# jluuser/PyTorch-VAE

Hardware: AMD Instinct MI355X
Metric: train images/sec @64x64x3 bs256 (curve tensors [B,64,6], SURVEY.md s0) (higher is better)
Workload: dtype f32; 1 GPU; C2: stage2_vq.yaml model with num_quantizers=1 K=512 D=64 N=64; full train step (fwd+loss+bwd+clip+AdamW+EMA), dropout 0.1, loss weights at epoch 100; per_gpu_batch=256, global_batch=256, seq_len=64, parallelism=dp1, hipgraph=True, params=43115078

## Files before the change

### pytorch-vae_amd/csrc/gemm.hip

```cpp
#include "common.h"
#include <type_traits>
#include <utility>
#include <vector>
#include <algorithm>

namespace {

constexpr int BM = 128, BN = 128;
constexpr int BK = 32;
template <int BKT> struct Tile {
    static constexpr int KC_LD = BKT + 4;
    static constexpr int A_TILE = BM * KC_LD;
    static constexpr int NLD = BKT / 8;
};

enum EpiMode {
    EPI_LINEAR = 0,
    EPI_RELU_DROP = 1,
    EPI_GELU = 2,
    EPI_DROP_RESID = 3,
    EPI_SIGMOID = 4,
    EPI_MUL_POSMASK = 5,
    EPI_MUL_GELUGRAD = 6,
    EPI_MUL_SIGGRAD = 7,
// ... 578 lines not shown
                        const float am = A[(size_t)(r + u * slices) * lda + m];
                        acc[m] += am * bv[u];
                        asum[m] += am;
                    }
        }
        for (; r < r1; r += slices) {
            const f32x4 bv = *reinterpret_cast<const f32x4*>(B + (size_t)r * ldb + q * 4);
#pragma unroll
            for (int m = 0; m < M; ++m) {
                    const float am = A[(size_t)r * lda + m];
                    acc[m] += am * bv;
                    asum[m] += am;
                }
        }
#pragma unroll
        for (int m = 0; m < M; ++m) {
                *reinterpret_cast<f32x4*>(red + ((size_t)sl * M + m) * N + q * 4) = acc[m];
                if (q == 0) red_rs[sl][m] = asum[m];
            }
    }
    __syncthreads();
    float* out = slab + (size_t)blockIdx.x * M * N;
    for (int i = threadIdx.x; i < M * nq; i += 256) {
        f32x4 v = *reinterpret_cast<const f32x4*>(red + (size_t)i * 4);
        for (int s2 = 1; s2 < slices; ++s2) v += *reinterpret_cast<const f32x4*>(red + (size_t)s2 * M * N + (size_t)i * 4);
        *reinterpret_cast<f32x4*>(out + (size_t)i * 4) = v;
    }
    if (rs && threadIdx.x < M) {
        float t = 0.f;
        for (int s2 = 0; s2 < slices; ++s2) t += red_rs[s2][threadIdx.x];
        rs[(size_t)blockIdx.x * M + threadIdx.x] = t;
    }
}

#include "gemm_dma.inc"
#include "gemm_p3.inc"

struct ProfRec { int slot; double flops; hipEvent_t e0, e1; };
bool g_prof_on = false;
std::vector<ProfRec> g_prof;
constexpr int PROF_MODES = 9;
constexpr int PROF_FAMILIES = 7;
inline int prof_slot(bool a_kc, bool b_kc, int mode_t, int family = 0) {
    return (family * 4 + (a_kc ? 2 : 0) + (b_kc ? 1 : 0)) * PROF_MODES + mode_t + 1;
}

template <bool A_KC, bool B_KC, int BKT, int MODE = -1>
int launch(const GemmArgs& g, int splits, hipStream_t stream) {
    static bool attr_set = false;
    const size_t smem = (size_t)4 * Tile<BKT>::A_TILE * sizeof(float);
    if (!attr_set) {
        hipError_t e = hipFuncSetAttribute(reinterpret_cast<const void*>(&gemm_f32_mfma<A_KC, B_KC, BKT, MODE>),
                                           hipFuncAttributeMaxDynamicSharedMemorySize, (int)smem);
        if (e != hipSuccess) {
            vqh_set_error(hipGetErrorString(e));
            return VQH_ERR_LAUNCH;
        }
        attr_set = true;
    }
    const int tiles = ((g.M + BM - 1) / BM) * ((g.N + BN - 1) / BN);
    dim3 grid(tiles, 1, splits);
    ProfRec rec{};
    if (g_prof_on) {
        rec.slot = prof_slot(A_KC, B_KC, MODE);
        rec.flops = 2.0 * g.M * g.N * g.K;
        if (hipEventCreate(&rec.e0) != hipSuccess || hipEventCreate(&rec.e1) != hipSuccess ||
            hipEventRecord(rec.e0, stream) != hipSuccess) {
            vqh_set_error("vqh_gemm: profiling events failed");
            return VQH_ERR_LAUNCH;
        }
    }
    hipLaunchKernelGGL((gemm_f32_mfma<A_KC, B_KC, BKT, MODE>), grid, dim3(256), smem, stream, g);
    VQH_LAUNCH_CHECK();
    if (g_prof_on) {
        if (hipEventRecord(rec.e1, stream) != hipSuccess) {
            vqh_set_error("vqh_gemm: profiling events failed");
            return VQH_ERR_LAUNCH;
        }
        g_prof.push_back(rec);
    }
    return VQH_OK;
}

template <bool A_KC, bool B_KC, int MODE, bool X3>
int launch_dma_impl(const GemmArgs& g, int splits, hipStream_t stream) {
    static bool attr_set = false;
    auto kern = X3 ? &gemm_f32_x3<A_KC, B_KC, MODE> : &gemm_f32_dma<A_KC, B_KC, MODE>;
    if (!attr_set) {
        hipError_t e = hipFuncSetAttribute(reinterpret_cast<const void*>(kern),
                                           hipFuncAttributeMaxDynamicSharedMemorySize, dma::LDS_BYTES);
        if (e != hipSuccess) {
            vqh_set_error(hipGetErrorString(e));
            return VQH_ERR_LAUNCH;
        }
        attr_set = true;
    }
    dim3 grid((g.M / dma::TBM) * (g.N / dma::TBN), 1, splits);
    ProfRec rec{};
    if (g_prof_on) {
        rec.slot = prof_slot(A_KC, B_KC, MODE, X3 ? 3 : 1);
        rec.flops = 2.0 * g.M * g.N * g.K;
        if (hipEventCreate(&rec.e0) != hipSuccess || hipEventCreate(&rec.e1) != hipSuccess ||
            hipEventRecord(rec.e0, stream) != hipSuccess) {
            vqh_set_error("vqh_gemm: profiling events failed");
            return VQH_ERR_LAUNCH;
        }
    }
    hipLaunchKernelGGL(kern, grid, dim3(256), dma::LDS_BYTES, stream, g);
    VQH_LAUNCH_CHECK();
    if (g_prof_on) {
        if (hipEventRecord(rec.e1, stream) != hipSuccess) {
            vqh_set_error("vqh_gemm: profiling events failed");
            return VQH_ERR_LAUNCH;
        }
        g_prof.push_back(rec);
    }
    return VQH_OK;
}

template <bool A_KC, bool B_KC, int MODE = -1>
int launch_dma(const GemmArgs& g, int splits, hipStream_t stream) {
    if (g.flags & 512) return launch_dma_impl<A_KC, B_KC, MODE, false>(g, splits, stream);
    return launch_dma_impl<A_KC, B_KC, MODE, true>(g, splits, stream);
}

}

extern "C" int vqh_gemm_profile_begin(void) {
    g_prof.clear();
    g_prof_on = true;
    return VQH_OK;
}
extern "C" int vqh_gemm_profile_end(double* out) {
    g_prof_on = false;
    if (out)
        for (int i = 0; i < PROF_FAMILIES * 4 * PROF_MODES * 3; ++i) out[i] = 0.0;
    int rc = VQH_OK;
    for (ProfRec& r : g_prof) {
        float ms = 0.f;
        if (hipEventSynchronize(r.e1) != hipSuccess || hipEventElapsedTime(&ms, r.e0, r.e1) != hipSuccess) {
            vqh_set_error("vqh_gemm_profile_end: event query failed");
            rc = VQH_ERR_LAUNCH;
        } else if (out) {
            out[r.slot * 3 + 0] += 1.0;
            out[r.slot * 3 + 1] += (double)ms * 1e-3;
            out[r.slot * 3 + 2] += r.flops;
        }
        (void)hipEventDestroy(r.e0);
        (void)hipEventDestroy(r.e1);
    }
    g_prof.clear();
    return rc;
}

extern "C" int vqh_reduce_slabs(const float* slabs, int S, long long stride, long long n, float* out, float beta,
                                hipStream_t stream);

static int g_gemm_flags = 1;
extern "C" int vqh_gemm_set_flags(int flags) {
#ifndef VQH_DIAG
    flags &= ~(2 | 4);
#endif
    const int old = g_gemm_flags; g_gemm_flags = flags; return old;
}

static int gemm_impl(int a_kcontig, int b_kcontig, int M, int N, int K, const float* A, int lda, const float* B,
                     int ldb, float* C, int ldc, const float* bias, int mode, const float* aux_in, float* aux_out,
                     int ldaux, float beta, const unsigned long long* rng_state, unsigned drop_site, float drop_p,
                     float* workspace, long long workspace_floats, float* rowsum, hipStream_t stream) {
    VQH_CHECK_ARG(M >= 0 && N >= 0 && K >= 0, "vqh_gemm: negative dimension");
    if (M == 0 || N == 0) return VQH_OK;
    VQH_CHECK_ARG(C && ((A && B) || K == 0), "vqh_gemm: null operand");
    VQH_CHECK_ARG(mode >= EPI_LINEAR && mode <= EPI_MUL_SIGGRAD, "vqh_gemm: unknown epilogue mode");
    VQH_CHECK_ARG(lda >= (a_kcontig ? K : M) && ldb >= (b_kcontig ? K : N) && ldc >= N, "vqh_gemm: leading dim too small");
    if (mode == EPI_GELU) VQH_CHECK_ARG(aux_out && ldaux >= N, "vqh_gemm: GELU epilogue needs aux_out");
    if (mode == EPI_DROP_RESID || mode >= EPI_MUL_POSMASK)
        VQH_CHECK_ARG(aux_in && ldaux >= N, "vqh_gemm: epilogue needs aux_in");
    VQH_CHECK_ARG(drop_p >= 0.f && drop_p < 1.f, "vqh_gemm: dropout p out of range");
    if (drop_p > 0.f && (mode == EPI_RELU_DROP || mode == EPI_DROP_RESID))
        VQH_CHECK_ARG(rng_state != nullptr, "vqh_gemm: dropout needs rng_state");

    GemmArgs g;
    g.A = A; g.B = B; g.C = C;
    g.M = M; g.N = N; g.K = K;
    g.lda = lda; g.ldb = ldb; g.ldc = ldc;
    g.vecA = ((reinterpret_cast<uintptr_t>(A) & 15) == 0 && (lda & 3) == 0) ? 1 : 0;
    g.vecB = ((reinterpret_cast<uintptr_t>(B) & 15) == 0 && (ldb & 3) == 0) ? 1 : 0;
    {
        uintptr_t al = reinterpret_cast<uintptr_t>(C) | reinterpret_cast<uintptr_t>(bias) | reinterpret_cast<uintptr_t>(aux_in) |
                       reinterpret_cast<uintptr_t>(aux_out);
        g.vecC = ((al & 15) == 0 && (ldc & 3) == 0 && ((aux_in || aux_out) ? (ldaux & 3) == 0 : true) && (N & 3) == 0) ? 1 : 0;
    }
    g.mode = mode; g.bias = bias; g.aux_in = aux_in; g.aux_out = aux_out; g.ldaux = ldaux; g.beta = beta;
    g.drop = make_drop(rng_state, drop_site, drop_p);
    g.ws = nullptr;
    g.rowsum = rowsum;
    g.rowsum_ws = nullptr;
    g.flags = g_gemm_flags;
    if (rowsum) VQH_CHECK_ARG(!a_kcontig && mode == EPI_LINEAR, "vqh_gemm_wgrad: row sums need the [K,M] A layout and a linear epilogue");

    if (!(g_gemm_flags & 64)) {
        auto al16 = [](const void* p_) { return (reinterpret_cast<uintptr_t>(p_) & 15) == 0; };
        if (mode == EPI_LINEAR && !rowsum && a_kcontig && b_kcontig && N <= SK_MAX && K >= 64 && (K & 3) == 0 &&
            (lda & 3) == 0 && (ldb & 3) == 0 && al16(A) && al16(B)) {
            int blocks = (M + 3) / 4;
            if (blocks > 2048) blocks = 2048;
#define SK_CASE(V) case V: hipLaunchKernelGGL(skinny_n_kernel<V>, dim3(blocks), dim3(256), 0, stream, A, lda, B, ldb, C, ldc, bias, beta, M, K); break
            switch (N) { SK_CASE(1); SK_CASE(2); SK_CASE(3); SK_CASE(4); SK_CASE(5); SK_CASE(6); SK_CASE(7); default: SK_CASE(8); }
#undef SK_CASE
            VQH_LAUNCH_CHECK();
            return VQH_OK;
        }
        if (mode == EPI_LINEAR && !rowsum && !bias && a_kcontig && !b_kcontig && K <= SK_MAX && K > 0 && N >= 64 &&
            (N & 3) == 0 && (ldb & 3) == 0 && (ldc & 3) == 0 && al16(B) && al16(C)) {
            const long long quads = (long long)M * (N >> 2);
            int blocks = (int)((quads + 255) / 256);
            if (blocks > 4096) blocks = 4096;
#define SK_CASE(V) case V: hipLaunchKernelGGL(skinny_k_kernel<V>, dim3(blocks), dim3(256), 0, stream, A, lda, B, ldb, C, ldc, beta, M, N); break
            switch (K) { SK_CASE(1); SK_CASE(2); SK_CASE(3); SK_CASE(4); SK_CASE(5); SK_CASE(6); SK_CASE(7); default: SK_CASE(8); }
#undef SK_CASE
            VQH_LAUNCH_CHECK();
            return VQH_OK;
        }
        if (mode == EPI_LINEAR && !a_kcontig && !b_kcontig && M <= SK_MAX && N >= 64 && (N & 3) == 0 && (ldb & 3) == 0 &&
            (ldc & 3) == 0 && al16(B) && al16(C) && al16(workspace) && !bias && workspace && K >= 256 && N <= 1024 &&
            256 % (N >> 2) == 0) {
            const int rows_per_block = 64;
            const int nblk = (K + rows_per_block - 1) / rows_per_block;
            const long long per = (long long)M * N + (rowsum ? M : 0);
            if ((long long)nblk * per <= workspace_floats && ldc == N) {
                float* rs_ws = rowsum ? workspace + (size_t)nblk * M * N : nullptr;
#define SK_CASE(V) case V: hipLaunchKernelGGL(skinny_m_kernel<V>, dim3(nblk), dim3(256), 0, stream, A, lda, B, ldb, workspace, rs_ws, N, K, rows_per_block); break
                switch (M) { SK_CASE(1); SK_CASE(2); SK_CASE(3); SK_CASE(4); SK_CASE(5); SK_CASE(6); SK_CASE(7); default: SK_CASE(8); }
#undef SK_CASE
                VQH_LAUNCH_CHECK();
                int rc2 = vqh_reduce_slabs(workspace, nblk, (long long)M * N, (long long)M * N, C, beta, stream);
                if (rc2 == VQH_OK && rowsum) rc2 = vqh_reduce_slabs(rs_ws, nblk, (long long)M, (long long)M, rowsum, beta, stream);
                return rc2;
            }
        }
    }

    if (!(g_gemm_flags & 128) && (M % dma::TBM) == 0 && (N % dma::TBN) == 0 && (K % dma::TBK) == 0 && K >= dma::TBK && g.vecA &&
        g.vecB && g.vecC && (!rowsum || (reinterpret_cast<uintptr_t>(workspace) & 15) == 0)) {
        const int tiles_d = (M / dma::TBM) * (N / dma::TBN);
        int splits_d = 1;
        if (workspace && mode == EPI_LINEAR && tiles_d < 192 && K >= 8 * dma::TBK) {
            splits_d = 256 / tiles_d;
            const int max_by_k = K / (4 * dma::TBK);
            if (splits_d > max_by_k) splits_d = max_by_k;
            const long long per = (long long)M * N + (rowsum ? M : 0);
            if ((long long)splits_d * per > workspace_floats) splits_d = (int)(workspace_floats / per);
            if (splits_d < 2) splits_d = 1;
        }
        int kchunk_d = ((K + splits_d - 1) / splits_d + dma::TBK - 1) / dma::TBK * dma::TBK;
        splits_d = (K + kchunk_d - 1) / kchunk_d;
        const bool pairs_fit = (long long)M * N / 2 < (1LL << 32);
        if (tiles_d * splits_d >= 96 && pairs_fit) {
            g.kchunk = kchunk_d;
            if (splits_d > 1) {
                g.ws = workspace;
                if (rowsum) g.rowsum_ws = workspace + (size_t)splits_d * M * N;
            }
            int rc;
            if (a_kcontig && b_kcontig) {
                if (splits_d == 1 && mode == EPI_DROP_RESID) rc = launch_dma<true, true, EPI_DROP_RESID>(g, splits_d, stream);
                else if (splits_d == 1 && mode == EPI_RELU_DROP) rc = launch_dma<true, true, EPI_RELU_DROP>(g, splits_d, stream);
                else if (splits_d == 1 && mode == EPI_GELU) rc = launch_dma<true, true, EPI_GELU>(g, splits_d, stream);
                else if (mode == EPI_LINEAR) rc = launch_dma<true, true, EPI_LINEAR>(g, splits_d, stream);
                else rc = launch_dma<true, true>(g, splits_d, stream);
            } else if (a_kcontig && !b_kcontig) {
                if (splits_d == 1 && mode == EPI_MUL_POSMASK) rc = launch_dma<true, false, EPI_MUL_POSMASK>(g, splits_d, stream);
                else if (splits_d == 1 && mode == EPI_MUL_GELUGRAD) rc = launch_dma<true, false, EPI_MUL_GELUGRAD>(g, splits_d, stream);
                else if (mode == EPI_LINEAR) rc = launch_dma<true, false, EPI_LINEAR>(g, splits_d, stream);
                else rc = launch_dma<true, false>(g, splits_d, stream);
            } else if (!a_kcontig && b_kcontig) {
                if (mode == EPI_LINEAR) rc = launch_dma<false, true, EPI_LINEAR>(g, splits_d, stream);
                else rc = launch_dma<false, true>(g, splits_d, stream);
            } else {
                if (mode == EPI_LINEAR) rc = launch_dma<false, false, EPI_LINEAR>(g, splits_d, stream);
                else rc = launch_dma<false, false>(g, splits_d, stream);
            }
            if (rc != VQH_OK) return rc;
            if (splits_d > 1) {
                const size_t total = (size_t)M * N;
                int blocks = (int)((total / 4 + 255) / 256);
                if (blocks > 4096) blocks = 4096;
                if (rowsum && blocks < (M + 255) / 256) blocks = (M + 255) / 256;
                hipLaunchKernelGGL(splitk_reduce_vec, dim3(blocks), dim3(256), 0, stream, workspace, splits_d, M, N, C, ldc, bias,
                                   beta, g.rowsum_ws, rowsum);
                VQH_LAUNCH_CHECK();
            }
            return VQH_OK;
        }
        g.ws = nullptr;
        g.rowsum_ws = nullptr;
    }

    const int tiles = ((M + BM - 1) / BM) * ((N + BN - 1) / BN);
    int splits = 1;
    if (workspace && mode == EPI_LINEAR && tiles < 256 && K >= 8 * BK) {
        splits = 512 / tiles;
        const int max_by_k = K / (4 * BK);
        if (splits > max_by_k) splits = max_by_k;
        const long long per = (long long)M * N + (rowsum ? M : 0);
        if ((long long)splits * per > workspace_floats) splits = (int)(workspace_floats / per);
        if (splits < 2) splits = 1;
    }
    int kchunk = ((K + splits - 1) / splits + BK - 1) / BK * BK;
    if (kchunk <= 0) kchunk = BK;
    splits = (K + kchunk - 1) / kchunk;
    if (splits < 1) splits = 1;
    g.kchunk = kchunk;
    if (splits > 1) {
        g.ws = workspace;
        if (rowsum) g.rowsum_ws = workspace + (size_t)splits * M * N;
    }

    int rc;
    if (splits == 1 && g.vecC && a_kcontig && b_kcontig && mode == EPI_DROP_RESID) {
        rc = launch<true, true, 32, EPI_DROP_RESID>(g, splits, stream);
    } else if (splits == 1 && g.vecC && a_kcontig && b_kcontig && mode == EPI_RELU_DROP) {
        rc = launch<true, true, 32, EPI_RELU_DROP>(g, splits, stream);
    } else if (splits == 1 && g.vecC && a_kcontig && b_kcontig && mode == EPI_GELU) {
        rc = launch<true, true, 32, EPI_GELU>(g, splits, stream);
    } else if (splits == 1 && g.vecC && a_kcontig && !b_kcontig && mode == EPI_MUL_POSMASK) {
        rc = launch<true, false, 32, EPI_MUL_POSMASK>(g, splits, stream);
    } else if (splits == 1 && g.vecC && a_kcontig && !b_kcontig && mode == EPI_MUL_GELUGRAD) {
        rc = launch<true, false, 32, EPI_MUL_GELUGRAD>(g, splits, stream);
    } else {
        if (a_kcontig && b_kcontig) rc = launch<true, true, 32>(g, splits, stream);
        else if (a_kcontig && !b_kcontig) rc = launch<true, false, 32>(g, splits, stream);
        else if (!a_kcontig && b_kcontig) rc = launch<false, true, 32>(g, splits, stream);
        else rc = launch<false, false, 32>(g, splits, stream);
    }
    if (rc != VQH_OK) return rc;
    if (splits > 1) {
        const size_t total = (size_t)M * N;
        int blocks = (int)((total + 255) / 256);
        if (blocks > 2048) blocks = 2048;
        if (rowsum && blocks < (M + 255) / 256) blocks = (M + 255) / 256;
// ... 522 lines not shown
```

### pytorch-vae_amd/csrc/gemm_dma.inc

```

namespace dma {
constexpr int TBM = 256, TBN = 128, TBK = 32;
constexpr int A_BYTES = TBM * TBK * 4, B_BYTES = TBN * TBK * 4, STAGE_BYTES = A_BYTES + B_BYTES;
constexpr int NSTAGE = 3, LDS_BYTES = NSTAGE * STAGE_BYTES;
constexpr int DMA_A = A_BYTES / 1024 / 4, DMA_B = B_BYTES / 1024 / 4, DMA_PER_WAVE = DMA_A + DMA_B;
constexpr int MI = 4, NJ = 2;
}

typedef float f32x2 __attribute__((ext_vector_type(2)));

typedef unsigned u32x2 __attribute__((ext_vector_type(2)));
typedef unsigned u32x4 __attribute__((ext_vector_type(4)));
typedef short s16x4 __attribute__((ext_vector_type(4)));
typedef __bf16 bf16x8 __attribute__((ext_vector_type(8)));

namespace x3 {
constexpr int A_PLANE = dma::TBM * dma::TBK * 2, B_PLANE = dma::TBN * dma::TBK * 2;
constexpr int B_OFF = 3 * A_PLANE;
constexpr int STAGE_BYTES = 3 * (A_PLANE + B_PLANE);
constexpr int LDS_BYTES = 2 * STAGE_BYTES;
constexpr int NU = 12, NUA = 8;
constexpr int NB = 8, G = 48, NSLOT = 96;
constexpr int BAR = 7 * NU;
constexpr int RS_OFF = 40960;
static_assert(LDS_BYTES <= dma::LDS_BYTES, "x3 stages must fit the launch's dynamic LDS");
}

template <class F, int... I>
__device__ __forceinline__ void static_for_impl(F&& f, std::integer_sequence<int, I...>) { (f(std::integral_constant<int, I>{}), ...); }
template <int N, class F>
__device__ __forceinline__ void static_for(F&& f) { static_for_impl(f, std::make_integer_sequence<int, N>{}); }

struct SplitUnit {
    float r0, r1, r2, r3;
    unsigned t0, t1, t2, t3;
    unsigned hp[2], mp[2], lp[2];
    template <int S> __device__ __forceinline__ void step(const f32x4& a) {
        if constexpr (S == 0) {
            asm volatile("v_cvt_pk_bf16_f32 %0, %6, %7\n\tv_cvt_pk_bf16_f32 %1, %8, %9\n\tv_lshlrev_b32 %2, 16, %0\n\t"
                         "v_and_b32 %3, 0xffff0000, %0\n\tv_sub_f32 %4, %6, %2\n\tv_sub_f32 %5, %7, %3"
                         : "=&v"(hp[0]), "=&v"(hp[1]), "=&v"(t0), "=&v"(t1), "=&v"(r0), "=&v"(r1)
                         : "v"(a[0]), "v"(a[1]), "v"(a[2]), "v"(a[3]) : "memory");
        } else if constexpr (S == 1) {
            asm volatile("v_lshlrev_b32 %0, 16, %6\n\tv_and_b32 %1, 0xffff0000, %6\n\tv_sub_f32 %2, %7, %0\n\t"
                         "v_sub_f32 %3, %8, %1\n\tv_cvt_pk_bf16_f32 %4, %9, %10\n\tv_cvt_pk_bf16_f32 %5, %2, %3"
                         : "=&v"(t2), "=&v"(t3), "=&v"(r2), "=&v"(r3), "=&v"(mp[0]), "=&v"(mp[1])
                         : "v"(hp[1]), "v"(a[2]), "v"(a[3]), "v"(r0), "v"(r1) : "memory");
        } else if constexpr (S == 2) {
            asm volatile("v_lshlrev_b32 %0, 16, %2\n\tv_and_b32 %1, 0xffff0000, %2" : "=&v"(t0), "=&v"(t1) : "v"(mp[0]) : "memory");
        } else if constexpr (S == 3) {
            asm volatile("v_sub_f32 %0, %0, %2\n\tv_sub_f32 %1, %1, %3" : "+v"(r0), "+v"(r1) : "v"(t0), "v"(t1) : "memory");
        } else if constexpr (S == 4) {
            asm volatile("v_lshlrev_b32 %0, 16, %6\n\tv_and_b32 %1, 0xffff0000, %6\n\tv_sub_f32 %2, %2, %0\n\t"
                         "v_sub_f32 %3, %3, %1\n\tv_cvt_pk_bf16_f32 %4, %7, %8\n\tv_cvt_pk_bf16_f32 %5, %2, %3"
                         : "=&v"(t2), "=&v"(t3), "+v"(r2), "+v"(r3), "=&v"(lp[0]), "=&v"(lp[1])
                         : "v"(mp[1]), "v"(r0), "v"(r1) : "memory");
        }
    }
    __device__ __forceinline__ void all(const f32x4& a) { step<0>(a); step<1>(a); step<2>(a); step<3>(a); step<4>(a); }
};

__device__ __forceinline__ void glds16_s(const char* ubase, unsigned voff, unsigned lds_byte_addr_uniform) {
    asm volatile("s_mov_b32 m0, %2\n\ts_nop 0\n\tglobal_load_lds_dwordx4 %0, %1"
                 :
                 : "v"(voff), "s"(ubase), "s"(lds_byte_addr_uniform)
                 : "memory");
}

__device__ __forceinline__ void glds16(const float* gptr, unsigned lds_byte_addr_uniform) {
    __builtin_amdgcn_global_load_lds(gptr, (__attribute__((address_space(3))) void*)(uintptr_t)lds_byte_addr_uniform, 16, 0, 0);
}

template <bool A_KC, bool B_KC, int MODE, bool X3 = false>
__device__ __forceinline__ void gemm_dma_tile(const GemmArgs& g, const int tile, const int zsplit) {
    using namespace dma;
    constexpr bool EA_KC = X3 ? true : A_KC, EB_KC = X3 ? true : B_KC;
    extern __shared__ __attribute__((aligned(1024))) unsigned char smem_dma[];
    const int tid = threadIdx.x, lane = tid & 63;
    const int wave = __builtin_amdgcn_readfirstlane(tid >> 6);
    const int wm = wave >> 1, wn = wave & 1;
    const int l31 = lane & 31, h = lane >> 5;

    const int tiles_n = g.N / TBN;
    const int m0 = (tile / tiles_n) * TBM, n0 = (tile % tiles_n) * TBN;
    const int kbeg = zsplit * g.kchunk;
    const int kend = min(g.K, kbeg + g.kchunk);
    const int nk = (kend - kbeg) / TBK;

    unsigned voff[DMA_PER_WAVE];
    unsigned dst[DMA_PER_WAVE];
#pragma unroll
    for (int i = 0; i < DMA_A; ++i) {
        const int j = wave + 4 * i;
        if (A_KC) {
            const int R = j * 8 + (lane >> 3), c = (lane & 7) ^ ((R >> 1) & 7);
            voff[i] = (unsigned)(((size_t)R * g.lda + c * 4) * 4);
        } else {
            voff[i] = (unsigned)(((size_t)j * g.lda + lane * 4) * 4);
        }
        dst[i] = j * 1024;
    }
#pragma unroll
    for (int i = 0; i < DMA_B; ++i) {
        const int j = wave + 4 * i;
        if (B_KC) {
            const int R = j * 8 + (lane >> 3), c = (lane & 7) ^ ((R >> 1) & 7);
            voff[DMA_A + i] = (unsigned)(((size_t)R * g.ldb + c * 4) * 4);
        } else {
            voff[DMA_A + i] = (unsigned)(((size_t)(2 * j + (lane >> 5)) * g.ldb + (lane & 31) * 4) * 4);
        }
        dst[DMA_A + i] = A_BYTES + j * 1024;
    }
    const char* baseA = reinterpret_cast<const char*>(A_KC ? g.A + (size_t)m0 * g.lda + kbeg : g.A + (size_t)kbeg * g.lda + m0);
    const char* baseB = reinterpret_cast<const char*>(B_KC ? g.B + (size_t)n0 * g.ldb + kbeg : g.B + (size_t)kbeg * g.ldb + n0);
    const size_t stepA = (A_KC ? (size_t)TBK : (size_t)TBK * g.lda) * 4;
    const size_t stepB = (B_KC ? (size_t)TBK : (size_t)TBK * g.ldb) * 4;
    const unsigned lds0 = (unsigned)(uintptr_t)smem_dma;

    const int sw = (l31 >> 1) & 7;
    unsigned offA[4], offB[4];
#pragma unroll
    for (int t = 0; t < 4; ++t) {
        offA[t] = A_KC ? (unsigned)((wm * 128 + l31) * 128 + (((2 * t + h) ^ sw) * 16))
                       : (unsigned)((8 * t + 4 * h) * (TBM * 4) + (wm * 128 + 4 * l31) * 4);
        offB[t] = A_BYTES + (B_KC ? (unsigned)((wn * 64 + l31) * 128 + (((2 * t + h) ^ sw) * 16))
                                  : (unsigned)((8 * t + 4 * h) * (TBN * 4) + (wn * 64 + 2 * l31) * 4));
    }

    f32x16 acc[MI][NJ];
#pragma unroll
    for (int i = 0; i < MI; ++i)
#pragma unroll
        for (int j = 0; j < NJ; ++j)
#pragma unroll
            for (int r = 0; r < 16; ++r) acc[i][j][r] = 0.f;

    f32x4 fa[2][4];
    f32x4 fbk[2][2];
    f32x2 fbr[2][4];
    const bool do_rowsum = (!A_KC) && (g.rowsum != nullptr) && (n0 == 0) && (X3 || wn == 0);
    float rs[4] = {0.f, 0.f, 0.f, 0.f};

    constexpr int NREAD = 4 + (B_KC ? 2 : 4);
    constexpr int NMF = 4 * MI * NJ;
    constexpr int GAP = NMF / (NREAD + 1);
    auto substep = [&](auto c_c, auto rt_c, auto v0_c, auto v1_c, int rstage, int kt_d, int dstage) {
        constexpr int c = decltype(c_c)::value, RT = decltype(rt_c)::value, V0 = decltype(v0_c)::value,
                      V1 = decltype(v1_c)::value, n = c ^ 1;
        const unsigned char* sb = smem_dma + rstage * STAGE_BYTES;
        const unsigned dsb = lds0 + dstage * STAGE_BYTES;
        if (do_rowsum) {
#pragma unroll
            for (int e = 0; e < 4; ++e)
#pragma unroll
                for (int i = 0; i < 4; ++i) rs[i] += fa[c][e][i];
        }
#pragma unroll
        for (int m = 0; m < NMF; ++m) {
            const int e = m / (MI * NJ), i = (m / NJ) % MI, j = m % NJ;
            const float av = A_KC ? fa[c][i][e] : fa[c][e][i];
            const float bv = B_KC ? fbk[c][j][e] : fbr[c][e][j];
            acc[i][j] = __builtin_amdgcn_mfma_f32_32x32x2f32(av, bv, acc[i][j], 0, 0, 0);
            if ((m % GAP) == 0 && m / GAP < NREAD) {
                const int d = m / GAP;
                if (d < 4) {
                    fa[n][d] = *reinterpret_cast<const f32x4*>(sb + offA[RT] + (A_KC ? d * 32 * 128 : d * TBM * 4));
                } else if (B_KC) {
                    fbk[n][d - 4] = *reinterpret_cast<const f32x4*>(sb + offB[RT] + (d - 4) * 32 * 128);
                } else {
                    fbr[n][d - 4] = *reinterpret_cast<const f32x2*>(sb + offB[RT] + (d - 4) * TBN * 4);
                }
            }
            if ((m % GAP) == GAP / 2 && V0 + m / GAP < V1) {
                const int v = V0 + m / GAP;
                const char* ub = (v < DMA_A) ? baseA + (size_t)kt_d * stepA : baseB + (size_t)kt_d * stepB;
                glds16_s(ub, voff[v], __builtin_amdgcn_readfirstlane(dsb + dst[v]));
            }
        }
#pragma unroll
        for (int m = 0; m < NMF; ++m) {
            __builtin_amdgcn_sched_group_barrier(0x008, 1, 0);
            if ((m % GAP) == 0 && m / GAP < NREAD) __builtin_amdgcn_sched_group_barrier(0x100, 1, 0);
            if ((m % GAP) == GAP / 2 && V0 + m / GAP < V1) __builtin_amdgcn_sched_group_barrier(0x020, 1, 0);
        }
    };
    auto read_first = [&](int rstage) {
        const unsigned char* sb = smem_dma + rstage * STAGE_BYTES;
#pragma unroll
        for (int d = 0; d < 4; ++d) fa[0][d] = *reinterpret_cast<const f32x4*>(sb + offA[0] + (A_KC ? d * 32 * 128 : d * TBM * 4));
        if (B_KC) {
#pragma unroll
            for (int d = 0; d < 2; ++d) fbk[0][d] = *reinterpret_cast<const f32x4*>(sb + offB[0] + d * 32 * 128);
        } else {
#pragma unroll
            for (int d = 0; d < 4; ++d) fbr[0][d] = *reinterpret_cast<const f32x2*>(sb + offB[0] + d * TBN * 4);
        }
    };
    auto issue_all = [&](int kt, int stage) {
        const unsigned sbb = lds0 + stage * STAGE_BYTES;
#pragma unroll
        for (int v = 0; v < DMA_PER_WAVE; ++v) {
            const char* ub = (v < DMA_A) ? baseA + (size_t)kt * stepA : baseB + (size_t)kt * stepB;
            glds16_s(ub, voff[v], __builtin_amdgcn_readfirstlane(sbb + dst[v]));
        }
    };

    const int c4 = (lane & 15) * 4;
    const int col = n0 + wn * 64 + c4;
    constexpr bool HAS_DROP = (MODE == EPI_RELU_DROP || MODE == EPI_DROP_RESID);
    constexpr bool HAS_AUX = (MODE == EPI_DROP_RESID || MODE > EPI_SIGMOID);
    unsigned dkey = 0;
    if (g.drop.p > 0.f && g.drop.rng_state) dkey = drop_key(g.drop, g.drop.rng_state[0], g.drop.rng_state[1]);
    unsigned dmask[4] = {0u, 0u, 0u, 0u};
    const unsigned pair0 = (unsigned)((((unsigned long long)(m0 + wm * 128 + (lane >> 4)) * g.N + col) >> 2) * 2);
    const unsigned g0 = pair0 * 0x9E3779B9U;
    const unsigned gstep = (unsigned)(2 * g.N) * 0x9E3779B9U;
    auto hash_quad = [&](int qi) {
        const unsigned gq = g0 + (unsigned)qi * gstep;
        const unsigned b0 = mix32(dkey ^ gq), b1 = mix32(dkey ^ (gq + 0x9E3779B9U));
        unsigned f4 = ((b0 & 0xffffu) >= g.drop.thr) ? 1u : 0u;
        f4 |= ((b0 >> 16) >= g.drop.thr) ? 2u : 0u;
        f4 |= ((b1 & 0xffffu) >= g.drop.thr) ? 4u : 0u;
        f4 |= ((b1 >> 16) >= g.drop.thr) ? 8u : 0u;
        const unsigned sh = f4 << ((qi & 7) * 4);
        const int w = qi >> 3;
#pragma unroll
        for (int k = 0; k < 4; ++k) dmask[k] |= (w == k) ? sh : 0u;
    };
    f32x4 auxr[32];
    auto load_aux_all = [&]() {
        const float* ap = g.aux_in + (size_t)(m0 + wm * 128 + (lane >> 4)) * g.ldaux + col;
#pragma unroll
        for (int q = 0; q < 32; ++q) auxr[q] = *reinterpret_cast<const f32x4*>(ap + (size_t)(q * 4) * g.ldaux);
    };

    using I0 = std::integral_constant<int, 0>;
    using I1 = std::integral_constant<int, 1>;
    using I2 = std::integral_constant<int, 2>;
    using I3 = std::integral_constant<int, 3>;
    using IH = std::integral_constant<int, DMA_PER_WAVE / 2>;
    using IF = std::integral_constant<int, DMA_PER_WAVE>;
    if constexpr (X3) {
        const unsigned vA = A_KC ? (unsigned)(((size_t)(8 * wave + (lane >> 3)) * g.lda + 4 * (lane & 7)) * 4)
                                 : (unsigned)(((size_t)(8 * wave) * g.lda + 4 * lane) * 4);
        const unsigned vB = B_KC ? (unsigned)(((size_t)(8 * wave + (lane >> 3)) * g.ldb + 4 * (lane & 7)) * 4)
                                 : (unsigned)(((size_t)(8 * wave + (lane >> 5)) * g.ldb + 4 * (lane & 31)) * 4);
        const size_t uA = (A_KC ? (size_t)32 * g.lda : (size_t)g.lda) * 4;
        const size_t uB = (B_KC ? (size_t)32 * g.ldb : (size_t)2 * g.ldb) * 4;
        unsigned wA[4], wB[2];
        {
            const int R = 8 * wave + (lane >> 3), c = (lane & 7) >> 1;
            const unsigned wkc = (unsigned)(R * 64 + ((c ^ ((R >> 2) & 3)) * 16) + (lane & 1) * 8);
#pragma unroll
            for (int x = 0; x < 4; ++x) wA[x] = A_KC ? wkc : (unsigned)((8 * wave) * 512 + (((lane >> 3) ^ x) * 64) + (lane & 7) * 8);
#pragma unroll
            for (int x = 0; x < 2; ++x)
                wB[x] = B_KC ? wkc
                             : (unsigned)((8 * wave + (lane >> 5)) * 256 + ((((lane >> 3) & 3) ^ ((2 * x + (lane >> 5)) & 3)) * 64) + (lane & 7) * 8);
        }
        unsigned rA[4], rB[2];
        {
            const int q = (lane & 15) >> 2, p = lane & 3, sub = (lane >> 4) & 1;
            if (A_KC) {
                const int R = wm * 128 + l31, f = (l31 >> 2) & 3;
                rA[0] = (unsigned)(R * 64 + ((h ^ f) * 16));
                rA[1] = (unsigned)(R * 64 + (((2 + h) ^ f) * 16));
                rA[2] = rA[3] = 0;
            } else {
#pragma unroll
                for (int i = 0; i < 4; ++i) rA[i] = (unsigned)((8 * h + q) * 512 + (((wm * 4 + i) ^ q) * 64) + (16 * sub + 4 * p) * 2);
            }
            if (B_KC) {
                const int R = wn * 64 + l31, f = (l31 >> 2) & 3;
                rB[0] = (unsigned)(R * 64 + ((h ^ f) * 16));
                rB[1] = (unsigned)(R * 64 + (((2 + h) ^ f) * 16));
            } else {
#pragma unroll
                for (int j = 0; j < 2; ++j) rB[j] = (unsigned)((8 * h + q) * 256 + (((wn * 2 + j) ^ q) * 64) + (16 * sub + 4 * p) * 2);
            }
        }
        f32x4 st[x3::NU];
        u32x4 xA[3][4];
        u32x4 xB[2][3][2];
        SplitUnit su;
        auto load_unit = [&](auto u_c, int kt) {
            constexpr int u = decltype(u_c)::value;
            if constexpr (u < x3::NUA) st[u] = *reinterpret_cast<const f32x4*>(baseA + (size_t)kt * stepA + (size_t)u * uA + vA);
            else st[u] = *reinterpret_cast<const f32x4*>(baseB + (size_t)kt * stepB + (size_t)(u - x3::NUA) * uB + vB);
        };
        auto write_unit = [&](auto u_c, auto pl_c, unsigned char* sb) {
            constexpr int u = decltype(u_c)::value, pl = decltype(pl_c)::value;
            const u32x2 v = pl == 0 ? u32x2{su.hp[0], su.hp[1]} : pl == 1 ? u32x2{su.mp[0], su.mp[1]} : u32x2{su.lp[0], su.lp[1]};
            if constexpr (u < x3::NUA) {
                constexpr int cst = A_KC ? u * 2048 : u * 512;
                *reinterpret_cast<u32x2*>(sb + pl * x3::A_PLANE + cst + wA[A_KC ? 0 : (u & 3)]) = v;
            } else {
                constexpr int i = u - x3::NUA;
                constexpr int cst = B_KC ? i * 2048 : 2 * i * 256;
                *reinterpret_cast<u32x2*>(sb + x3::B_OFF + pl * x3::B_PLANE + cst + wB[B_KC ? 0 : (i & 1)]) = v;
            }
        };
        auto read_A = [&](auto pl_c, auto i_c, auto g_c, const unsigned char* sb) -> u32x4 {
            constexpr int pl = decltype(pl_c)::value, i = decltype(i_c)::value, gg = decltype(g_c)::value;
            if constexpr (A_KC) {
                return *reinterpret_cast<const u32x4*>(sb + pl * x3::A_PLANE + i * 2048 + rA[gg]);
            } else {
                const unsigned a0 = (unsigned)(uintptr_t)(sb + pl * x3::A_PLANE + (16 * gg) * 512 + rA[i]);
                const s16x4 lo = __builtin_amdgcn_ds_read_tr16_b64_v4i16((__attribute__((address_space(3))) s16x4*)(uintptr_t)a0);
                const s16x4 hi = __builtin_amdgcn_ds_read_tr16_b64_v4i16((__attribute__((address_space(3))) s16x4*)(uintptr_t)(a0 + 4 * 512));
                const u32x2 l2 = __builtin_bit_cast(u32x2, lo), h2 = __builtin_bit_cast(u32x2, hi);
                return u32x4{l2[0], l2[1], h2[0], h2[1]};
            }
        };
        auto read_B = [&](auto pl_c, auto j_c, auto g_c, const unsigned char* sb) -> u32x4 {
            constexpr int pl = decltype(pl_c)::value, j = decltype(j_c)::value, gg = decltype(g_c)::value;
            if constexpr (B_KC) {
                return *reinterpret_cast<const u32x4*>(sb + x3::B_OFF + pl * x3::B_PLANE + j * 2048 + rB[gg]);
            } else {
                const unsigned a0 = (unsigned)(uintptr_t)(sb + x3::B_OFF + pl * x3::B_PLANE + (16 * gg) * 256 + rB[j]);
                const s16x4 lo = __builtin_amdgcn_ds_read_tr16_b64_v4i16((__attribute__((address_space(3))) s16x4*)(uintptr_t)a0);
                const s16x4 hi = __builtin_amdgcn_ds_read_tr16_b64_v4i16((__attribute__((address_space(3))) s16x4*)(uintptr_t)(a0 + 4 * 256));
                const u32x2 l2 = __builtin_bit_cast(u32x2, lo), h2 = __builtin_bit_cast(u32x2, hi);
                return u32x4{l2[0], l2[1], h2[0], h2[1]};
            }
        };
        auto aux_one = [&](auto q_c) {
            constexpr int q = decltype(q_c)::value;
            auxr[q] = *reinterpret_cast<const f32x4*>(g.aux_in + (size_t)(m0 + wm * 128 + (lane >> 4) + q * 4) * g.ldaux + col);
        };
        if (nk > 0) {
            static_for<x3::NU>([&](auto u_c) { load_unit(u_c, 0); });
            if (HAS_DROP && g.drop.p > 0.f && !g.ws) {
#pragma unroll
                for (int qi = 0; qi < 32; ++qi) hash_quad(qi);
            }
            static_for<x3::NU>([&](auto u_c) {
                constexpr int u = decltype(u_c)::value;
                if (do_rowsum && u < x3::NUA) {
#pragma unroll
                    for (int e = 0; e < 4; ++e) rs[e] += st[u][e];
                }
                su.all(st[u]);
                write_unit(u_c, I0{}, smem_dma);
                write_unit(u_c, I1{}, smem_dma);
                write_unit(u_c, I2{}, smem_dma);
                load_unit(u_c, nk > 1 ? 1 : 0);
            });
            asm volatile("s_waitcnt lgkmcnt(0)" ::: "memory");
            __builtin_amdgcn_s_barrier();
            static_for<4>([&](auto i_c) { xA[0][decltype(i_c)::value] = read_A(I0{}, i_c, I0{}, smem_dma); });
            static_for<6>([&](auto x_c) {
                constexpr int x = decltype(x_c)::value;
                xB[0][x / 2][x % 2] = read_B(std::integral_constant<int, x / 2>{}, std::integral_constant<int, x % 2>{}, I0{}, smem_dma);
            });
            auto kstep = [&](auto last_c, const int kt) {
                constexpr bool LAST = decltype(last_c)::value;
                const unsigned char* rstg = smem_dma + (kt & 1) * x3::STAGE_BYTES;
                unsigned char* wstg = smem_dma + ((kt & 1) ^ 1) * x3::STAGE_BYTES;
                const int kt_ld = min(kt + 2, nk - 1);
                const bool want_aux = LAST && HAS_AUX && !g.ws;
                static_for<x3::NSLOT>([&](auto m_c) {
                    constexpr int m = decltype(m_c)::value;
                    constexpr int gg = m / x3::G, mm = m % x3::G, pi = mm / x3::NB, b = mm % x3::NB, i = b / 2, j = b % 2;
                    constexpr int pa = (pi < 3) ? 0 : (pi < 5) ? 1 : 2;
                    constexpr int pb = (pi == 0 || pi == 3 || pi == 5) ? 0 : (pi == 1 || pi == 4) ? 1 : 2;
                    acc[i][j] = __builtin_amdgcn_mfma_f32_32x32x16_bf16(__builtin_bit_cast(bf16x8, xA[pa][i]),
                                                                        __builtin_bit_cast(bf16x8, xB[gg][pb][j]), acc[i][j], 0, 0, 0);
                    if constexpr (m < 8 && m % 2 == 0) xA[1][m / 2] = read_A(I1{}, std::integral_constant<int, m / 2>{}, I0{}, rstg);
                    if constexpr (m >= 8 && m < 16 && m % 2 == 0) xA[2][(m - 8) / 2] = read_A(I2{}, std::integral_constant<int, (m - 8) / 2>{}, I0{}, rstg);
                    if constexpr (m >= 16 && m < 28 && m % 2 == 0) {
                        constexpr int x = (m - 16) / 2;
                        xB[1][x / 2][x % 2] = read_B(std::integral_constant<int, x / 2>{}, std::integral_constant<int, x % 2>{}, I1{}, rstg);
                    }
                    if constexpr (m >= 28 && m < 44 && m % 4 == 0) xA[0][(m - 28) / 4] = read_A(I0{}, std::integral_constant<int, (m - 28) / 4>{}, I1{}, rstg);
                    if constexpr (m >= 48 && m < 56 && m % 2 == 0) xA[1][(m - 48) / 2] = read_A(I1{}, std::integral_constant<int, (m - 48) / 2>{}, I1{}, rstg);
                    if constexpr (m >= 56 && m < 64 && m % 2 == 0) xA[2][(m - 56) / 2] = read_A(I2{}, std::integral_constant<int, (m - 56) / 2>{}, I1{}, rstg);
                    if constexpr (!LAST) {
                        if constexpr (m >= x3::BAR && m < x3::BAR + 4) xA[0][m - x3::BAR] = read_A(I0{}, std::integral_constant<int, m - x3::BAR>{}, I0{}, wstg);
                        if constexpr (m >= x3::BAR + 4 && m < x3::BAR + 10) {
                            constexpr int x = m - x3::BAR - 4;
                            xB[0][x / 2][x % 2] = read_B(std::integral_constant<int, x / 2>{}, std::integral_constant<int, x % 2>{}, I0{}, wstg);
                        }
                        if constexpr (m < x3::BAR) {
                            constexpr int u = m / 7, ph = m % 7;
                            using U = std::integral_constant<int, u>;
                            if constexpr (ph == 0) {
                                if (do_rowsum && u < x3::NUA) {
#pragma unroll
                                    for (int e = 0; e < 4; ++e) rs[e] += st[u][e];
                                }
                                su.template step<0>(st[u]);
                            }
                            if constexpr (ph == 1) su.template step<1>(st[u]);
                            if constexpr (ph == 2) { su.template step<2>(st[u]); write_unit(U{}, I0{}, wstg); }
                            if constexpr (ph == 3) { su.template step<3>(st[u]); write_unit(U{}, I1{}, wstg); }
                            if constexpr (ph == 4) load_unit(U{}, kt_ld);
                            if constexpr (ph == 5) su.template step<4>(st[u]);
                            if constexpr (ph == 6) write_unit(U{}, I2{}, wstg);
                        }
                        if constexpr (m == x3::BAR - 1) {
                            asm volatile("s_waitcnt lgkmcnt(0)" ::: "memory");
                            __builtin_amdgcn_s_barrier();
                        }
                    } else if constexpr (HAS_AUX) {
                        if constexpr (m % 3 == 0) {
                            if (want_aux) aux_one(std::integral_constant<int, m / 3>{});
                        }
                    }
                    __builtin_amdgcn_sched_barrier(0);
                });
            };
            for (int kt = 0; kt < nk - 1; ++kt) kstep(std::false_type{}, kt);
            kstep(std::true_type{}, nk - 1);
            __builtin_amdgcn_s_barrier();
        } else if (HAS_AUX && !g.ws) {
            load_aux_all();
        }
    } else
    if (nk > 0) {
        issue_all(0, 0);
        issue_all(nk > 1 ? 1 : 0, 1);
        if (HAS_DROP && g.drop.p > 0.f && !g.ws) {
#pragma unroll
            for (int qi = 0; qi < 32; ++qi) hash_quad(qi);
        }
        asm volatile("s_waitcnt vmcnt(%0)" ::"n"(DMA_PER_WAVE) : "memory");
        __builtin_amdgcn_s_barrier();
        read_first(0);
        int stage = 0;
        for (int kt = 0; kt < nk; ++kt) {
            const int nxt = (stage == 2) ? 0 : stage + 1;
            const int nx2 = (nxt == 2) ? 0 : nxt + 1;
            if (HAS_AUX && !g.ws && kt == nk - 1) load_aux_all();
            substep(I0{}, I1{}, I0{}, I0{}, stage, 0, 0);
            substep(I1{}, I2{}, I0{}, I0{}, stage, 0, 0);
            asm volatile("s_waitcnt vmcnt(0)" ::: "memory");
            __builtin_amdgcn_s_barrier();
            const int ktd = min(kt + 2, nk - 1);
            substep(I0{}, I3{}, I0{}, IH{}, stage, ktd, nx2);
            substep(I1{}, I0{}, IH{}, IF{}, nxt, ktd, nx2);
            stage = nxt;
        }
        asm volatile("s_waitcnt vmcnt(0)" ::: "memory");
        __builtin_amdgcn_s_barrier();
    } else if (HAS_AUX && !g.ws) {
        load_aux_all();
    }

    if (X3 && do_rowsum) {
        float* rsb = reinterpret_cast<float*>(smem_dma + x3::RS_OFF);
        *reinterpret_cast<f32x4*>(rsb + wave * TBM + 4 * lane) = f32x4{rs[0], rs[1], rs[2], rs[3]};
        __builtin_amdgcn_s_barrier();
        if (wave == 0) {
            f32x4 t = *reinterpret_cast<const f32x4*>(rsb + 4 * lane);
#pragma unroll
            for (int w = 1; w < 4; ++w) t += *reinterpret_cast<const f32x4*>(rsb + w * TBM + 4 * lane);
            const int row = m0 + 4 * lane;
            if (g.rowsum_ws) {
                *reinterpret_cast<f32x4*>(g.rowsum_ws + (size_t)zsplit * g.M + row) = t;
            } else {
#pragma unroll
                for (int i = 0; i < 4; ++i) g.rowsum[row + i] = (g.beta != 0.f) ? g.beta * g.rowsum[row + i] + t[i] : t[i];
            }
        }
    } else
    if (do_rowsum) {
#pragma unroll
        for (int i = 0; i < 4; ++i) rs[i] += __shfl_xor(rs[i], 32, 64);
        if (h == 0) {
            const int row = m0 + wm * 128 + 4 * l31;
            if (g.rowsum_ws) {
                *reinterpret_cast<f32x4*>(g.rowsum_ws + (size_t)zsplit * g.M + row) = f32x4{rs[0], rs[1], rs[2], rs[3]};
            } else {
#pragma unroll
                for (int i = 0; i < 4; ++i)
                    g.rowsum[row + i] = (g.beta != 0.f) ? g.beta * g.rowsum[row + i] + rs[i] : rs[i];
            }
        }
    }

    const int mode = (MODE >= 0) ? MODE : g.mode;
    constexpr int EP_LD = 68;
    float* ep = reinterpret_cast<float*>(smem_dma) + wave * (32 * EP_LD);
    float* slab = g.ws ? g.ws + (size_t)zsplit * g.M * g.N : nullptr;
    if constexpr (X3 && MODE == EPI_LINEAR) {
        if (!(g.flags & 2048)) {
            const size_t ldo = slab ? (size_t)g.N : (size_t)g.ldc;
            float* obase = slab ? slab : g.C;
#pragma unroll
            for (int j = 0; j < NJ; ++j) {
                const int cj = n0 + wn * 64 + j * 32 + l31;
                const float bj = (g.bias && !slab) ? g.bias[cj] : 0.f;
                float* cp = obase + (size_t)(m0 + wm * 128 + 4 * h) * ldo + cj;
                if (!slab && g.beta != 0.f) {
#pragma unroll
                    for (int i = 0; i < MI; ++i)
#pragma unroll
                        for (int r = 0; r < 16; ++r) {
                            float* q = cp + (size_t)(i * 32 + (r & 3) + 8 * (r >> 2)) * ldo;
                            *q = acc[i][j][r] + bj + g.beta * *q;
                        }
                } else {
#pragma unroll
                    for (int i = 0; i < MI; ++i)
#pragma unroll
                        for (int r = 0; r < 16; ++r) cp[(size_t)(i * 32 + (r & 3) + 8 * (r >> 2)) * ldo] = acc[i][j][r] + bj;
                }
            }
            return;
        }
    }
    f32x4 bias4 = {0.f, 0.f, 0.f, 0.f};
    if (mode <= EPI_SIGMOID && g.bias && !slab) bias4 = *reinterpret_cast<const f32x4*>(g.bias + col);
#pragma unroll
    for (int grp = 0; grp < 4; ++grp) {
        __builtin_amdgcn_wave_barrier();
#pragma unroll
        for (int q = 0; q < 16; ++q) {
            int rr, i, r;
            if (EA_KC) { i = grp; r = q; rr = (q & 3) + 8 * (q >> 2) + 4 * h; }
            else { i = q >> 2; r = 4 * grp + (q & 3); rr = 4 * ((q & 3) + 4 * h) + i; }
            if (EB_KC) {
                ep[rr * EP_LD + l31] = acc[i][0][r];
                ep[rr * EP_LD + 32 + l31] = acc[i][1][r];
            } else {
                *reinterpret_cast<f32x2*>(ep + rr * EP_LD + 2 * l31) = f32x2{acc[i][0][r], acc[i][1][r]};
            }
        }
        __builtin_amdgcn_s_waitcnt(0xC07F);
        __builtin_amdgcn_wave_barrier();
        constexpr int EPI_UNROLL = (MODE >= 0) ? 8 : 1;
#pragma unroll EPI_UNROLL
        for (int it = 0; it < 8; ++it) {
            const int rl = it * 4 + (lane >> 4);
            const int row = m0 + wm * 128 + grp * 32 + rl;
            f32x4 v = *reinterpret_cast<const f32x4*>(ep + rl * EP_LD + c4);
            if (slab) {
                *reinterpret_cast<f32x4*>(slab + (size_t)row * g.N + col) = v;
                continue;
            }
            float* cptr = g.C + (size_t)row * g.ldc + col;
            if (mode <= EPI_SIGMOID) {
                v += bias4;
                if (mode == EPI_RELU_DROP || mode == EPI_DROP_RESID) {
                    if (mode == EPI_RELU_DROP)
#pragma unroll
                        for (int e = 0; e < 4; ++e) v[e] = fmaxf(v[e], 0.f);
                    if (g.drop.p > 0.f) {
                        if (HAS_DROP) {
#pragma unroll
                            for (int e = 0; e < 4; ++e) v[e] = ((dmask[grp] >> (it * 4 + e)) & 1u) ? v[e] * g.drop.scale : 0.f;
                        } else {
                            float f[4];
                            drop4(g.drop, dkey, ((unsigned long long)row * g.N + col) >> 2, f);
#pragma unroll
                            for (int e = 0; e < 4; ++e) v[e] *= f[e];
                        }
                    }
                    if (mode == EPI_DROP_RESID)
                        v += HAS_AUX ? auxr[grp * 8 + it] : *reinterpret_cast<const f32x4*>(g.aux_in + (size_t)row * g.ldaux + col);
                } else if (mode == EPI_GELU) {
                    *reinterpret_cast<f32x4*>(g.aux_out + (size_t)row * g.ldaux + col) = v;
#pragma unroll
                    for (int e = 0; e < 4; ++e) v[e] = gelu_erf(v[e]);
                } else if (mode == EPI_SIGMOID) {
#pragma unroll
                    for (int e = 0; e < 4; ++e) v[e] = 1.f / (1.f + __expf(-v[e]));
                }
            } else {
                const f32x4 a = HAS_AUX ? auxr[grp * 8 + it] : *reinterpret_cast<const f32x4*>(g.aux_in + (size_t)row * g.ldaux + col);
                if (mode == EPI_MUL_POSMASK) {
#pragma unroll
                    for (int e = 0; e < 4; ++e) v[e] = (a[e] > 0.f) ? v[e] * g.drop.scale : 0.f;
                } else if (mode == EPI_MUL_GELUGRAD) {
#pragma unroll
                    for (int e = 0; e < 4; ++e) v[e] *= gelu_erf_grad(a[e]);
                } else {
#pragma unroll
                    for (int e = 0; e < 4; ++e) v[e] *= a[e] * (1.f - a[e]);
                }
            }
            if (g.beta != 0.f) v += g.beta * *reinterpret_cast<const f32x4*>(cptr);
            *reinterpret_cast<f32x4*>(cptr) = v;
        }
        __builtin_amdgcn_s_waitcnt(0xC07F);
    }
}

template <bool A_KC, bool B_KC, int MODE>
__global__ __launch_bounds__(256, 1) void gemm_f32_dma(const GemmArgs g) {
    const int nx = gridDim.x, nt = nx * gridDim.z, lin = blockIdx.z * nx + blockIdx.x;
    const int q = nt >> 3, r = nt & 7, x = lin & 7, j = lin >> 3;
    const int v = (x < r ? x * (q + 1) : r * (q + 1) + (x - r) * q) + j;
    gemm_dma_tile<A_KC, B_KC, MODE>(g, v % nx, v / nx);
}

template <bool A_KC, bool B_KC, int MODE>
__global__ __launch_bounds__(256, 1) void gemm_f32_x3(const GemmArgs g) {
    const int nx = gridDim.x, nt = nx * gridDim.z, lin = blockIdx.z * nx + blockIdx.x;
    const int q = nt >> 3, r = nt & 7, x = lin & 7, j = lin >> 3;
    const int v = (x < r ? x * (q + 1) : r * (q + 1) + (x - r) * q) + j;
    gemm_dma_tile<A_KC, B_KC, MODE, true>(g, v % nx, v / nx);
}

constexpr int GROUP_MAX = 8;
struct GemmGroupArgs {
    int n;
    int wg_begin[GROUP_MAX + 1];
    int tiles[GROUP_MAX];
    GemmArgs p[GROUP_MAX];
};

__device__ __forceinline__ int group_logical_id() {
    const int nt = gridDim.x, lin = blockIdx.x;
    const int q = nt >> 3, r = nt & 7, x = lin & 7, j = lin >> 3;
    return (x < r ? x * (q + 1) : r * (q + 1) + (x - r) * q) + j;
}

__global__ __launch_bounds__(256, 1) void gemm_f32_dma_group(const GemmGroupArgs G) {
    const int v = ((G.p[0].flags & 1) && !(G.p[0].flags & 1024)) ? group_logical_id() : (int)blockIdx.x;
    int p = 0;
    while (p + 1 < G.n && v >= G.wg_begin[p + 1]) ++p;
    const int local = v - G.wg_begin[p];
    const int tiles = G.tiles[p];
    gemm_dma_tile<false, false, EPI_LINEAR>(G.p[p], local % tiles, local / tiles);
}
__global__ __launch_bounds__(256, 1) void gemm_f32_x3_group(const GemmGroupArgs G) {
    const int v = ((G.p[0].flags & 1) && !(G.p[0].flags & 1024)) ? group_logical_id() : (int)blockIdx.x;
    int p = 0;
    while (p + 1 < G.n && v >= G.wg_begin[p + 1]) ++p;
    const int local = v - G.wg_begin[p];
    const int tiles = G.tiles[p];
    gemm_dma_tile<false, false, EPI_LINEAR, true>(G.p[p], local % tiles, local / tiles);
}
```

Measured before the change: 9289 images/s.

## Add register-direct epilogue for x3 GEMM ReLU-dropout and GELU modes

For the x3 (bf16x3 split) DMA GEMM path with RELU_DROP or GELU epilogues, results are now written straight from accumulator registers to global memory instead of being staged through LDS. The dropout hash is computed per unit and interleaved into the last k-step's MFMA schedule, with masks exchanged between lane pairs via DPP. The final barrier is skipped. The old LDS-staged path stays available as a separate kernel behind a flag. A second flag can force the DMA path for small tile counts. This trades the LDS round trip and barrier for uncoalesced strided global stores, plus extra registers and hash work inside the main loop.

```diff
diff --git a/pytorch-vae_amd/csrc/gemm.hip b/pytorch-vae_amd/csrc/gemm.hip
--- a/pytorch-vae_amd/csrc/gemm.hip
+++ b/pytorch-vae_amd/csrc/gemm.hip
@@ -684,10 +684,13 @@
     return VQH_OK;
 }
 
-template <bool A_KC, bool B_KC, int MODE, bool X3>
+template <bool A_KC, bool B_KC, int MODE, bool X3, bool STAGED = false>
 int launch_dma_impl(const GemmArgs& g, int splits, hipStream_t stream) {
     static bool attr_set = false;
-    auto kern = X3 ? &gemm_f32_x3<A_KC, B_KC, MODE> : &gemm_f32_dma<A_KC, B_KC, MODE>;
+    void (*kern)(const GemmArgs);
+    if constexpr (!X3) kern = &gemm_f32_dma<A_KC, B_KC, MODE>;
+    else if constexpr (STAGED) kern = &gemm_f32_x3_staged<A_KC, B_KC, MODE>;
+    else kern = &gemm_f32_x3<A_KC, B_KC, MODE>;
     if (!attr_set) {
         hipError_t e = hipFuncSetAttribute(reinterpret_cast<const void*>(kern),
                                            hipFuncAttributeMaxDynamicSharedMemorySize, dma::LDS_BYTES);
@@ -723,6 +726,9 @@
 template <bool A_KC, bool B_KC, int MODE = -1>
 int launch_dma(const GemmArgs& g, int splits, hipStream_t stream) {
     if (g.flags & 512) return launch_dma_impl<A_KC, B_KC, MODE, false>(g, splits, stream);
+    if constexpr (x3_register_epilogue(MODE)) {
+        if (g.flags & 2048) return launch_dma_impl<A_KC, B_KC, MODE, true, true>(g, splits, stream);
+    }
     return launch_dma_impl<A_KC, B_KC, MODE, true>(g, splits, stream);
 }
 
@@ -858,7 +864,7 @@
         int kchunk_d = ((K + splits_d - 1) / splits_d + dma::TBK - 1) / dma::TBK * dma::TBK;
         splits_d = (K + kchunk_d - 1) / kchunk_d;
         const bool pairs_fit = (long long)M * N / 2 < (1LL << 32);
-        if (tiles_d * splits_d >= 96 && pairs_fit) {
+        if ((tiles_d * splits_d >= 96 || (g_gemm_flags & 4096)) && pairs_fit) {
             g.kchunk = kchunk_d;
             if (splits_d > 1) {
                 g.ws = workspace;
diff --git a/pytorch-vae_amd/csrc/gemm_dma.inc b/pytorch-vae_amd/csrc/gemm_dma.inc
--- a/pytorch-vae_amd/csrc/gemm_dma.inc
+++ b/pytorch-vae_amd/csrc/gemm_dma.inc
@@ -8,6 +8,7 @@
 }
 
 typedef float f32x2 __attribute__((ext_vector_type(2)));
+constexpr bool x3_register_epilogue(int mode) { return mode == EPI_RELU_DROP || mode == EPI_GELU; }
 
 typedef unsigned u32x2 __attribute__((ext_vector_type(2)));
 typedef unsigned u32x4 __attribute__((ext_vector_type(4)));
@@ -71,7 +72,7 @@
     __builtin_amdgcn_global_load_lds(gptr, (__attribute__((address_space(3))) void*)(uintptr_t)lds_byte_addr_uniform, 16, 0, 0);
 }
 
-template <bool A_KC, bool B_KC, int MODE, bool X3 = false>
+template <bool A_KC, bool B_KC, int MODE, bool X3 = false, bool STAGED = false>
 __device__ __forceinline__ void gemm_dma_tile(const GemmArgs& g, const int tile, const int zsplit) {
     using namespace dma;
     constexpr bool EA_KC = X3 ? true : A_KC, EB_KC = X3 ? true : B_KC;
@@ -233,6 +234,25 @@
 #pragma unroll
         for (int q = 0; q < 32; ++q) auxr[q] = *reinterpret_cast<const f32x4*>(ap + (size_t)(q * 4) * g.ldaux);
     };
+    constexpr bool REG_EPI = X3 && !STAGED && x3_register_epilogue(MODE);
+    float bj2[2] = {0.f, 0.f};
+    auto load_bias2 = [&]() {
+        if (REG_EPI && g.bias) {
+            bj2[0] = g.bias[n0 + wn * 64 + l31];
+            bj2[1] = g.bias[n0 + wn * 64 + 32 + l31];
+        }
+    };
+    const unsigned par = lane & 1;
+    const unsigned gp0 = (unsigned)(((unsigned long long)(m0 + wm * 128 + 4 * h + par) * g.N + n0 + wn * 64 + l31) >> 1) * 0x9E3779B9U;
+    const unsigned nhalf = (unsigned)g.N >> 1;
+    auto hash_unit = [&](const int e) {
+        const int i = e >> 4, j = (e >> 3) & 1, t = e & 7;
+        const unsigned rowoff = (unsigned)(i * 32 + ((2 * t) & 3) + 8 * (t >> 1));
+        const unsigned b = mix32(dkey ^ (gp0 + (rowoff * nhalf + 16u * j) * 0x9E3779B9U));
+        const unsigned lo = ((b & 0xffffu) >= g.drop.thr) ? 1u : 0u, hi = ((b >> 16) >= g.drop.thr) ? 1u : 0u;
+        if (e < 32) { dmask[0] = dmask[0] + dmask[0] + lo; dmask[2] = dmask[2] + dmask[2] + hi; }
+        else { dmask[1] = dmask[1] + dmask[1] + lo; dmask[3] = dmask[3] + dmask[3] + hi; }
+    };
 
     using I0 = std::integral_constant<int, 0>;
     using I1 = std::integral_constant<int, 1>;
@@ -331,8 +351,13 @@
         if (nk > 0) {
             static_for<x3::NU>([&](auto u_c) { load_unit(u_c, 0); });
             if (HAS_DROP && g.drop.p > 0.f && !g.ws) {
-#pragma unroll
-                for (int qi = 0; qi < 32; ++qi) hash_quad(qi);
+                if constexpr (!REG_EPI) {
+#pragma unroll
+                    for (int qi = 0; qi < 32; ++qi) hash_quad(qi);
+                } else if (nk == 1) {
+#pragma unroll 1
+                    for (int e = 0; e < 64; ++e) hash_unit(e);
+                }
             }
             static_for<x3::NU>([&](auto u_c) {
                 constexpr int u = decltype(u_c)::value;
@@ -355,6 +380,7 @@
             });
             auto kstep = [&](auto last_c, const int kt) {
                 constexpr bool LAST = decltype(last_c)::value;
+                const bool want_hash = LAST && REG_EPI && HAS_DROP && g.drop.p > 0.f && nk > 1;
                 const unsigned char* rstg = smem_dma + (kt & 1) * x3::STAGE_BYTES;
                 unsigned char* wstg = smem_dma + ((kt & 1) ^ 1) * x3::STAGE_BYTES;
                 const int kt_ld = min(kt + 2, nk - 1);
@@ -402,6 +428,10 @@
                             asm volatile("s_waitcnt lgkmcnt(0)" ::: "memory");
                             __builtin_amdgcn_s_barrier();
                         }
+                    } else if constexpr (REG_EPI) {
+                        if constexpr (HAS_DROP && m % 3 == 1) {
+                            if (want_hash) { hash_unit(2 * (m / 3)); hash_unit(2 * (m / 3) + 1); }
+                        }
                     } else if constexpr (HAS_AUX) {
                         if constexpr (m % 3 == 0) {
                             if (want_aux) aux_one(std::integral_constant<int, m / 3>{});
@@ -411,11 +441,13 @@
                 });
             };
             for (int kt = 0; kt < nk - 1; ++kt) kstep(std::false_type{}, kt);
+            load_bias2();
             kstep(std::true_type{}, nk - 1);
-            __builtin_amdgcn_s_barrier();
+            if constexpr (!REG_EPI) __builtin_amdgcn_s_barrier();
         } else if (HAS_AUX && !g.ws) {
             load_aux_all();
         }
+        if (nk <= 0) load_bias2();
     } else
     if (nk > 0) {
         issue_all(0, 0);
@@ -510,6 +542,49 @@
             return;
         }
     }
+    if constexpr (REG_EPI) {
+        {
+            unsigned fr[2][2] = {{0u, 0u}, {0u, 0u}};
+            if (HAS_DROP && g.drop.p > 0.f) {
+#pragma unroll
+                for (int w = 0; w < 2; ++w) {
+                    const unsigned own = par ? dmask[2 + w] : dmask[w], oth = par ? dmask[w] : dmask[2 + w];
+                    const unsigned got = (unsigned)__builtin_amdgcn_update_dpp(0, (int)oth, 0xB1, 0xf, 0xf, true);
+                    fr[0][w] = par ? got : own;
+                    fr[1][w] = par ? own : got;
+                }
+            }
+            float* cp = g.C + (size_t)(m0 + wm * 128 + 4 * h) * g.ldc + n0 + wn * 64 + l31;
+            auto store_all = [&](auto beta_c) {
+                constexpr bool BETA = decltype(beta_c)::value;
+#pragma unroll
+                for (int i = 0; i < MI; ++i)
+#pragma unroll
+                    for (int j = 0; j < NJ; ++j)
+#pragma unroll
+                        for (int r = 0; r < 16; ++r) {
+                            const int rl = i * 32 + (r & 3) + 8 * (r >> 2);
+                            const int e = (2 * i + j) * 8 + (r >> 1);
+                            float v = acc[i][j][r];
+                            v += bj2[j];
+                            if constexpr (MODE == EPI_RELU_DROP) {
+                                v = fmaxf(v, 0.f);
+                                if (g.drop.p > 0.f) v = ((fr[r & 1][e >> 5] >> (31 - (e & 31))) & 1u) ? v * g.drop.scale : 0.f;
+                            } else {
+                                g.aux_out[(size_t)(m0 + wm * 128 + 4 * h + rl) * g.ldaux + n0 + wn * 64 + j * 32 + l31] = v;
+                                v = gelu_erf(v);
+                            }
+                            float* q = cp + (size_t)rl * g.ldc + j * 32;
+                            if constexpr (BETA) v += g.beta * *q;
+                            *q = v;
+                            if ((r & 3) == 3) __builtin_amdgcn_sched_barrier(0);
+                        }
+            };
+            if (g.beta != 0.f) store_all(std::true_type{});
+            else store_all(std::false_type{});
+            return;
+        }
+    }
     f32x4 bias4 = {0.f, 0.f, 0.f, 0.f};
     if (mode <= EPI_SIGMOID && g.bias && !slab) bias4 = *reinterpret_cast<const f32x4*>(g.bias + col);
 #pragma unroll
@@ -602,6 +677,13 @@
     const int v = (x < r ? x * (q + 1) : r * (q + 1) + (x - r) * q) + j;
     gemm_dma_tile<A_KC, B_KC, MODE, true>(g, v % nx, v / nx);
 }
+template <bool A_KC, bool B_KC, int MODE>
+__global__ __launch_bounds__(256, 1) void gemm_f32_x3_staged(const GemmArgs g) {
+    const int nx = gridDim.x, nt = nx * gridDim.z, lin = blockIdx.z * nx + blockIdx.x;
+    const int q = nt >> 3, r = nt & 7, x = lin & 7, j = lin >> 3;
+    const int v = (x < r ? x * (q + 1) : r * (q + 1) + (x - r) * q) + j;
+    gemm_dma_tile<A_KC, B_KC, MODE, true, true>(g, v % nx, v / nx);
+}
 
 constexpr int GROUP_MAX = 8;
 struct GemmGroupArgs {
```

Measured after the change: 9332 images/s (median of 6 runs). Within noise of the previous version (+0.5%).
